# HilaManor/AudioEditingCode

Measured on AMD Instinct MI355X. Metric: edited-clips/sec (200-step inv+edit, 10 s@16 kHz), higher is better.
Workload: dtype f32

## Files before the change

audioeditingcode_amd/csrc/conv_gemm_x6.hip:

```cpp
#include "cg_params.h"

typedef __bf16 bf16x8 __attribute__((ext_vector_type(8)));
typedef __bf16 bf16x2 __attribute__((ext_vector_type(2)));
typedef float f32x2 __attribute__((ext_vector_type(2)));

int launch_conv_gemm_x6(const aed_op* op, hipStream_t s);

constexpr int X6_BK = 16;

__device__ __forceinline__ void x6_split_pair(float x0, float x1, unsigned& h, unsigned& m, unsigned& l) {
    h = __builtin_bit_cast(unsigned, __builtin_convertvector((f32x2){x0, x1}, bf16x2));
    float r0 = x0 - __uint_as_float(h << 16);
    float r1 = x1 - __uint_as_float(h & 0xffff0000u);
    asm volatile("" : "+v"(r0), "+v"(r1));
    m = __builtin_bit_cast(unsigned, __builtin_convertvector((f32x2){r0, r1}, bf16x2));
    float q0 = r0 - __uint_as_float(m << 16);
    float q1 = r1 - __uint_as_float(m & 0xffff0000u);
    asm volatile("" : "+v"(q0), "+v"(q1));
    l = __builtin_bit_cast(unsigned, __builtin_convertvector((f32x2){q0, q1}, bf16x2));
}

typedef unsigned u32x4 __attribute__((ext_vector_type(4)));
constexpr unsigned X6_OOB = 0x80000000u;

template <int G, int NM, int NV>
__device__ __forceinline__ void x6_hints() {
    if constexpr (G < NM) {
        constexpr int v = (NV * (G + 1)) / NM - (NV * G) / NM;
        if constexpr (v > 0) __builtin_amdgcn_sched_group_barrier(0x002, v, 0);
        __builtin_amdgcn_sched_group_barrier(0x008, 1, 0);
        x6_hints<G + 1, NM, NV>();
    }
}

template <int BM, int BN, int WROWS, int WCOLS, int DEPTH, bool PLAIN, int SCHED, int NTERMS, int BK = X6_BK>
__global__ __launch_bounds__(64 * WROWS * WCOLS, 2) void conv_gemm_x6_kernel(CGParams p) {
    constexpr int NT = 64 * WROWS * WCOLS;
    constexpr int WM = BM / WROWS, WN = BN / WCOLS;
    constexpr int TM = WM / 32, TN = WN / 32;
    constexpr int TPR = BK / 4;
    constexpr int RPP = NT / TPR;
    constexpr int PA = BM / RPP, PB = BN / RPP;
    constexpr int PQ = BK / 8;
    constexpr int X6_ROWQ = 3 * PQ + 1;
    constexpr int KB = BK / 16;
    constexpr int STAGE = (BM + BN) * X6_ROWQ;
    static_assert(BK == 16 || BK == 32, "chunk width");
    static_assert(TM >= 1 && TN >= 1 && PA >= 1 && PB >= 1, "tile");
    static_assert(BM % RPP == 0 && BN % RPP == 0, "loader passes");

    __shared__ uint4 lds[2 * STAGE];
    const unsigned nx = gridDim.x, ny = gridDim.y, bz = blockIdx.z, gz = gridDim.z;
    const unsigned orig = blockIdx.y * nx + blockIdx.x;

    const int tid = threadIdx.x;
    const int lane = tid & 63;
    const int wave = tid >> 6;
    const int wr = wave / WCOLS, wc = wave % WCOLS;
    int tile_y = (int)(orig / nx), tile_x = (int)(orig - (unsigned)tile_y * nx);
    if (gz == 1) {
        const unsigned nwg = nx * ny;
        const unsigned xcd = orig & 7u, q = nwg >> 3, r = nwg & 7u;
        const unsigned id = (xcd < r ? xcd * (q + 1) : r * (q + 1) + (xcd - r) * q) + (orig >> 3);
        if (p.gm > 1) {
            const unsigned per_group = (unsigned)p.gm * nx;
            const unsigned g = id / per_group, first = g * (unsigned)p.gm;
            const unsigned gsz = min((unsigned)p.gm, ny - first);
            const unsigned within = id - g * per_group;
            tile_x = (int)(within / gsz);
            tile_y = (int)(first + (within - (unsigned)tile_x * gsz));
        } else {
            tile_y = (int)(id / nx);
            tile_x = (int)(id - (unsigned)tile_y * nx);
        }
    }
    const int m0 = tile_y * BM;
    const int n0 = tile_x * BN;

    int kc_begin = 0, kc_end = p.nchunks;
    if (p.ksplit > 1) {
        const int per = (p.nchunks + p.ksplit - 1) / p.ksplit;
        kc_begin = (int)bz * per;
        kc_end = min(p.nchunks, kc_begin + per);
    }

    const int lrow = tid / TPR;
    const int lq = tid % TPR;
    const int lcol = lq * 4;

    int ay0[PA], ax0[PA];
    unsigned abase[PA], abase2[PA];
    bool avalid[PA];
#pragma unroll
    for (int q = 0; q < PA; ++q) {
        const int m = m0 + lrow + RPP * q;
        avalid[q] = m < p.M;
        const int mm = avalid[q] ? m : 0;
        int b = 0, r = mm, oy = mm, ox = 0;
        if (p.rpb != p.M || p.OW != 1) {
            b = mm / p.rpb;
            r = mm - b * p.rpb;
            oy = r / p.OW;
            ox = r - oy * p.OW;
        }
        ay0[q] = oy * p.stride - p.pad_h;
        ax0[q] = ox * p.stride - p.pad_w;
        abase[q] = (unsigned)b * (unsigned)p.a_bs + lcol;
        abase2[q] = (unsigned)b * (unsigned)p.a_bs2 + lcol;
    }
    unsigned wbase[PB];
    bool wvalid[PB];
#pragma unroll
    for (int q = 0; q < PB; ++q) {
        const int n = n0 + lrow + RPP * q;
        wvalid[q] = n < p.N;
        wbase[q] = (unsigned)(wvalid[q] ? n : 0) * (unsigned)p.K + lcol;
    }
    const int vIH = p.vIH, vIW = p.vIW;
    int pf_cg, pf_sub, pf_ty, pf_tx;
    const int gq = p.kgroup / BK;
    if (kc_begin == 0) {
        pf_cg = pf_sub = pf_ty = pf_tx = 0;
    } else {
        const int per_group = p.KH * p.KW * gq;
        const int g = kc_begin / per_group;
        const int rem = kc_begin - g * per_group;
        const int tap = rem / gq;
        pf_cg = g * p.kgroup;
        pf_sub = rem - tap * gq;
        pf_ty = tap / p.KW;
        pf_tx = tap - pf_ty * p.KW;
    }

    float4 rbuf_a[DEPTH][PA], rbuf_b[DEPTH][PB];
    float ln_s1[PA], ln_s2[PA];
#pragma unroll
    for (int q = 0; q < PA; ++q) { ln_s1[q] = 0.f; ln_s2[q] = 0.f; }

    const __amdgpu_buffer_rsrc_t srd_a = __builtin_amdgcn_make_buffer_rsrc((void*)p.A, 0, 0x7ffffff0, 0x00020000);
    const __amdgpu_buffer_rsrc_t srd_a2 = __builtin_amdgcn_make_buffer_rsrc((void*)(p.A2 ? p.A2 : p.A), 0, 0x7ffffff0, 0x00020000);
    const __amdgpu_buffer_rsrc_t srd_w = __builtin_amdgcn_make_buffer_rsrc((void*)p.W, 0, 0x7ffffff0, 0x00020000);
    auto as_f4 = [](u32x4 v) {
        return make_float4(__uint_as_float(v.x), __uint_as_float(v.y), __uint_as_float(v.z), __uint_as_float(v.w));
    };
    auto prefetch = [&](int kc, float4 (&ra)[PA], float4 (&rb)[PB]) {
        int c0 = pf_cg + pf_sub * BK;
        const int dy = pf_ty * p.dil_h, dx = pf_tx * p.dil_w;
        const unsigned k0 = (unsigned)((pf_ty * p.KW + pf_tx) * p.Cin + c0);
        pf_sub += 1;
        const bool wrap = pf_sub == gq;
        pf_sub = wrap ? 0 : pf_sub;
        pf_tx += wrap ? 1 : 0;
        const bool wrap2 = pf_tx == p.KW;
        pf_tx = wrap2 ? 0 : pf_tx;
        pf_ty += wrap2 ? 1 : 0;
        const bool wrap3 = pf_ty == p.KH;
        pf_ty = wrap3 ? 0 : pf_ty;
        pf_cg += wrap3 ? p.kgroup : 0;
        const bool second = p.C1 > 0 && c0 >= p.C1;
        c0 -= second ? p.C1 : 0;
        const unsigned ld = second ? (unsigned)p.lda2 : (unsigned)p.lda;
        const bool dead = kc >= kc_end;
#pragma unroll
        for (int q = 0; q < PA; ++q) {
            const int iy = ay0[q] + dy, ix = ax0[q] + dx;
            const bool ok = avalid[q] & ((unsigned)iy < (unsigned)vIH) & ((unsigned)ix < (unsigned)vIW) & !dead;
            const unsigned base = second ? abase2[q] : abase[q];
            const unsigned off = (base + (unsigned)((iy >> p.up) * p.IW + (ix >> p.up)) * ld + (unsigned)c0) * 4u;
            ra[q] = as_f4(__builtin_amdgcn_raw_buffer_load_b128(second ? srd_a2 : srd_a, ok ? off : X6_OOB, 0, 0));
        }
#pragma unroll
        for (int q = 0; q < PB; ++q)
            rb[q] = as_f4(__builtin_amdgcn_raw_buffer_load_b128(
                srd_w, (wvalid[q] & !dead) ? (wbase[q] + k0) * 4u : X6_OOB, 0, 0));
    };

    auto put_row = [&](uint4* st, int row, float4 v, bool is_w = false) {
        unsigned h0, m0_, l0, h1, m1, l1;
#ifdef X6_DIAG_NOSPLIT
        if (X6_DIAG_NOSPLIT == 2 || is_w) {
            h0 = __builtin_bit_cast(unsigned, __builtin_convertvector((f32x2){v.x, v.y}, bf16x2));
            h1 = __builtin_bit_cast(unsigned, __builtin_convertvector((f32x2){v.z, v.w}, bf16x2));
            m0_ = l0 = h0;
            m1 = l1 = h1;
        } else
#endif
        {
            x6_split_pair(v.x, v.y, h0, m0_, l0);
            x6_split_pair(v.z, v.w, h1, m1, l1);
        }
        uint2* dst = reinterpret_cast<uint2*>(st + row * X6_ROWQ) + lq;
        dst[0] = make_uint2(h0, h1);
        dst[2 * PQ] = make_uint2(m0_, m1);
        dst[4 * PQ] = make_uint2(l0, l1);
    };

    auto stage_write = [&](uint4* st, const float4 (&ra)[PA], const float4 (&rb)[PB]) {
#pragma unroll
        for (int q = 0; q < PA; ++q) {
            float4 v = ra[q];
            if constexpr (!PLAIN) {
                if (p.ln_mode) {
                    ln_s1[q] += (v.x + v.y) + (v.z + v.w);
                    ln_s2[q] += (v.x * v.x + v.y * v.y) + (v.z * v.z + v.w * v.w);
                }
                if (p.in_act) {
                    v.x = in_transform(v.x, p.in_act, p.in_slope);
                    v.y = in_transform(v.y, p.in_act, p.in_slope);
                    v.z = in_transform(v.z, p.in_act, p.in_slope);
                    v.w = in_transform(v.w, p.in_act, p.in_slope);
                }
            }
            put_row(st, lrow + RPP * q, v);
        }
#pragma unroll
        for (int q = 0; q < PB; ++q) put_row(st, BM + lrow + RPP * q, rb[q], true);
    };

    f32x16 acc[TM][TN];
#pragma unroll
    for (int a = 0; a < TM; ++a)
#pragma unroll
        for (int b = 0; b < TN; ++b)
#pragma unroll
            for (int r = 0; r < 16; ++r) acc[a][b][r] = 0.f;

    const int fi = lane & 31;
    const int fh = lane >> 5;
    const int a_frag = (wr * WM + fi) * X6_ROWQ + fh;
    const int b_frag = (BM + wc * WN + fi) * X6_ROWQ + fh;

    bf16x8 af[TM][3], bw[TN][3];
    auto load_frags = [&](const uint4* st, int kb, bf16x8 (&fa)[TM][3], bf16x8 (&fb)[TN][3]) {
#pragma unroll
        for (int a = 0; a < TM; ++a)
#pragma unroll
            for (int pl = 0; pl < 3; ++pl)
                fa[a][pl] = __builtin_bit_cast(bf16x8, st[a_frag + a * 32 * X6_ROWQ + PQ * pl + 2 * kb]);
#pragma unroll
        for (int b = 0; b < TN; ++b)
#pragma unroll
            for (int pl = 0; pl < 3; ++pl)
                fb[b][pl] = __builtin_bit_cast(bf16x8, st[b_frag + b * 32 * X6_ROWQ + PQ * pl + 2 * kb]);
    };
    auto do_mfmas = [&](const bf16x8 (&fa)[TM][3], const bf16x8 (&fb)[TN][3]) {
        constexpr int TA[6] = {0, 2, 1, 0, 1, 0};
        constexpr int TB[6] = {2, 0, 1, 1, 0, 0};
#pragma unroll
        for (int t = 6 - NTERMS; t < 6; ++t)
#pragma unroll
            for (int a = 0; a < TM; ++a)
#pragma unroll
                for (int b = 0; b < TN; ++b)
                    acc[a][b] = __builtin_amdgcn_mfma_f32_32x32x16_bf16(fa[a][TA[t]], fb[b][TB[t]], acc[a][b], 0, 0, 0);
    };
    auto hints = [&]() {
        if constexpr (SCHED == 1) {
            constexpr int NM = TM * TN * NTERMS * KB;
            x6_hints<0, NM, NM * (((PA + PB) * 22 + 40 + NM - 1) / NM)>();
        }
    };

#pragma unroll
    for (int d = 0; d < DEPTH; ++d) prefetch(kc_begin + d, rbuf_a[d], rbuf_b[d]);
    stage_write(lds, rbuf_a[0], rbuf_b[0]);
    prefetch(kc_begin + DEPTH, rbuf_a[0], rbuf_b[0]);
    __syncthreads();
    int cur = 0;
    for (int kc0 = kc_begin; kc0 < kc_end; kc0 += DEPTH) {
#pragma unroll
        for (int d = 0; d < DEPTH; ++d) {
            const int kc = kc0 + d;
            const int sl = (d + 1) % DEPTH;
            load_frags(lds + cur * STAGE, 0, af, bw);
            stage_write(lds + (cur ^ 1) * STAGE, rbuf_a[sl], rbuf_b[sl]);
            prefetch(kc + 1 + DEPTH, rbuf_a[sl], rbuf_b[sl]);
            do_mfmas(af, bw);
            if constexpr (KB == 2) {
                bf16x8 af2[TM][3], bw2[TN][3];
                load_frags(lds + cur * STAGE, 1, af2, bw2);
                do_mfmas(af2, bw2);
            }
            hints();
            __syncthreads();
            cur ^= 1;
        }
    }

    float* ln_stat = reinterpret_cast<float*>(lds);
#include "cg_epilogue.h"
}

template <int BM, int BN, int WR, int WC, int DEPTH, bool DIAG, int BK = X6_BK>
static int x6_launch(const CGParams& p, bool plain, int sched, int terms, hipStream_t s) {
    dim3 grid(aed_cdiv(p.N, BN), aed_cdiv(p.M, BM), p.ksplit);
    dim3 block(64 * WR * WC);
#define X6_GO(PL, SC, NT_) hipLaunchKernelGGL((conv_gemm_x6_kernel<BM, BN, WR, WC, DEPTH, PL, SC, NT_, BK>), grid, block, 0, s, p)
    if (terms == 3) {
        if constexpr (DIAG) {
            if (plain) { X6_GO(true, 1, 3); return 0; }
        }
        AED_REQUIRE(false, "conv_gemm_x6: the three-term diagnostic exists for tiles 1 and 8 with a plain A operand");
    }
    if (!plain) X6_GO(false, 1, 6);
    else if (sched) X6_GO(true, 1, 6);
    else X6_GO(true, 0, 6);
#undef X6_GO
    return 0;
}

int launch_conv_gemm_x6(const aed_op* op, hipStream_t s) {
    const int32_t* i = op->i;
    const int Cin = i[11];
    int cfg = i[29];
    const long long batch = i[0] / (i[9] * i[10] > 0 ? i[9] * i[10] : 1);
    const bool fits = (Cin % X6_BK == 0) && (i[3] % 4 == 0) && ((uintptr_t)op->p[0] % 16 == 0) &&
                      ((uintptr_t)op->p[1] % 16 == 0) && cfg < 10 && cfg != 5 && cfg != 6 && cfg != 7 && i[36] == 0 &&
                      i[37] == 0 && i[38] <= 1 && i[39] == 0 &&
                      batch * i[20] + (long long)i[7] * i[8] * i[3] < (1LL << 29) && (long long)i[1] * i[2] < (1LL << 29) &&
                      (i[32] == 0 || batch * i[34] + (long long)i[7] * i[8] * i[33] < (1LL << 29));
    if (!fits) {
        if (cfg == 8 || cfg == 9) {
            aed_op fp32_op = *op;
            fp32_op.i[29] = 1;
            return launch_conv_gemm(&fp32_op, s);
        }
        return launch_conv_gemm(op, s);
    }
    const bool wide = (op->flags & 256) && (cfg == 8 || cfg == 9) && Cin % 32 == 0 && !(op->flags & 16);
    CGParams p;
    int rc = cg_fill_params(op, p, wide ? 32 : X6_BK);
    if (rc) return rc;
    if (p.ksplit > (p.K + 31) / 32) p.ksplit = (p.K + 31) / 32;
    if (cfg == 0) {
        const int cus = aed_num_cus();
        auto blocks = [&](int bm, int bn) { return (long)aed_cdiv(p.M, bm) * aed_cdiv(p.N, bn) * p.ksplit; };
        if (p.N >= 512 && p.N % 256 == 0 && blocks(128, 256) >= 2L * cus) cfg = 9;
        else if (blocks(256, 128) >= 2L * cus && p.N >= 128) cfg = 8;
        else if (blocks(128, 128) >= (long)cus && p.N >= 128) cfg = 1;
        else if (blocks(128, 64) >= 2L * cus) cfg = 2;
        else cfg = 4;
    }
    if (!(op->flags & 1024) && p.ksplit <= 1) {
        static const int BMs[10] = {0, 128, 128, 64, 64, 0, 0, 0, 256, 128}, BNs[10] = {0, 128, 64, 128, 64, 0, 0, 0, 128, 256};
        const int nx = aed_cdiv(p.N, BNs[cfg]), ny = aed_cdiv(p.M, BMs[cfg]);
        const int resident = ((aed_num_cus() >> ((op->flags >> 16) & 3)) / 8) * ((cfg == 8 || cfg == 9) ? 1 : 2);
        if (nx > 1 && ny > 1) {
            int g = 1;
            while (g * 2 <= ny && (long)(g * 2) * (g * 2) * BMs[cfg] <= (long)resident * BNs[cfg]) g *= 2;
            if (resident / g < nx) p.gm = g;
            if (op->flags & 0x3800) p.gm = 1 << ((op->flags >> 11) & 7);
        }
    }
    const bool plain = p.in_act == 0 && p.ln_mode == 0;
    const int sched = (op->flags & 8) ? 1 : 0;
    const int terms = (op->flags & 16) ? 3 : 6;
    if (p.geglu) AED_REQUIRE(cfg == 1 || cfg == 3 || cfg == 8 || cfg == 9, "conv_gemm_x6: the GEGLU epilogue needs 64-wide wave tiles (cfg %d)", cfg);
    switch (cfg) {
        case 1: rc = x6_launch<128, 128, 2, 2, 2, true>(p, plain, sched, terms, s); break;
        case 2: rc = x6_launch<128, 64, 2, 2, 2, false>(p, plain, sched, terms, s); break;
        case 3: rc = x6_launch<64, 128, 2, 2, 2, false>(p, plain, sched, terms, s); break;
        case 4: rc = x6_launch<64, 64, 2, 2, 2, false>(p, plain, sched, terms, s); break;
        case 8: rc = wide && terms == 6 ? x6_launch<256, 128, 4, 2, 2, false, 32>(p, plain, sched, terms, s)
                                        : x6_launch<256, 128, 4, 2, 2, true>(p, plain, sched, terms, s); break;
        case 9: rc = wide && terms == 6 ? x6_launch<128, 256, 2, 4, 2, false, 32>(p, plain, sched, terms, s)
                                        : x6_launch<128, 256, 2, 4, 2, false>(p, plain, sched, terms, s); break;
        default: AED_REQUIRE(false, "conv_gemm_x6: bad tile cfg %d", cfg);
    }
    if (rc) return rc;
    AED_CHECK_HIP(hipGetLastError());
    if (p.ksplit > 1) return launch_splitk_reduce(op, s);
    return 0;
}
```

audioeditingcode_amd/tile_table_x6_cus64.py:

```python
TILE_TABLE = {
    (2, 512, 128, 0): (10, 1),
    (2, 512, 512, 0): (12, 1),
    (2, 8320, 512, 0): (10, 1),
    (128, 384, 3456, 0): (104, 16),
    (128, 640, 384, 0): (10, 1),
    (128, 640, 640, 0): (10, 1),
    (128, 640, 1024, 0): (104, 8),
    (128, 640, 1280, 0): (104, 8),
    (128, 640, 3200, 0): (104, 8),
    (128, 640, 3456, 0): (103, 16),
    (128, 640, 5760, 0): (103, 16),
    (128, 640, 9216, 0): (103, 16),
    (128, 640, 11520, 0): (103, 16),
    (128, 1920, 640, 0): (15, 1),
    (128, 5120, 640, 1): (103, 1),
    (512, 256, 2304, 0): (103, 8),
    (512, 384, 256, 0): (10, 1),
    (512, 384, 384, 0): (10, 1),
    (512, 384, 640, 0): (10, 1),
    (512, 384, 768, 0): (10, 1),
    (512, 384, 1024, 0): (104, 4),
    (512, 384, 1920, 0): (103, 8),
    (512, 384, 2304, 0): (103, 8),
    (512, 384, 3456, 0): (103, 8),
    (512, 384, 5760, 0): (103, 8),
    (512, 384, 6912, 0): (103, 8),
    (512, 384, 9216, 0): (103, 8),
    (512, 640, 5760, 0): (103, 8),
    (512, 1152, 384, 0): (104, 1),
    (512, 3072, 384, 1): (103, 1),
    (2048, 128, 1152, 0): (103, 4),
    (2048, 256, 128, 0): (104, 1),
    (2048, 256, 256, 0): (104, 1),
    (2048, 256, 384, 0): (104, 1),
    (2048, 256, 512, 0): (104, 1),
    (2048, 256, 640, 0): (104, 1),
    (2048, 256, 1152, 0): (103, 2),
    (2048, 256, 1280, 0): (103, 2),
    (2048, 256, 2304, 0): (103, 4),
    (2048, 256, 3456, 0): (103, 4),
    (2048, 256, 4608, 0): (103, 8),
    (2048, 256, 5760, 0): (103, 8),
    (2048, 384, 3456, 0): (103, 2),
    (2048, 768, 256, 0): (103, 1),
    (2048, 2048, 256, 1): (109, 1),
    (8192, 8, 1152, 0): (10, 1),
    (8192, 128, 72, 0): (4, 1),
    (8192, 128, 256, 0): (103, 1),
    (8192, 128, 384, 0): (103, 1),
    (8192, 128, 1152, 0): (103, 1),
    (8192, 128, 2304, 0): (103, 1),
    (8192, 128, 3456, 0): (103, 1),
    (8192, 256, 2304, 0): (109, 1),
}
```

audioeditingcode_amd/tile_table_x6_cus64_b1.py:

```python
TILE_TABLE = {
    (1, 512, 128, 0): (10, 1),
    (1, 512, 512, 0): (10, 1),
    (1, 8320, 512, 0): (10, 1),
    (64, 384, 3456, 0): (104, 16),
    (64, 640, 384, 0): (12, 1),
    (64, 640, 640, 0): (12, 1),
    (64, 640, 1024, 0): (11, 1),
    (64, 640, 1280, 0): (11, 1),
    (64, 640, 3200, 0): (104, 16),
    (64, 640, 3456, 0): (104, 16),
    (64, 640, 5760, 0): (103, 32),
    (64, 640, 9216, 0): (103, 32),
    (64, 640, 11520, 0): (104, 16),
    (64, 1920, 640, 0): (10, 1),
    (64, 5120, 640, 1): (13, 1),
    (256, 256, 2304, 0): (104, 8),
    (256, 384, 256, 0): (10, 1),
    (256, 384, 384, 0): (10, 1),
    (256, 384, 640, 0): (10, 1),
    (256, 384, 768, 0): (10, 1),
    (256, 384, 1024, 0): (104, 8),
    (256, 384, 1920, 0): (104, 8),
    (256, 384, 2304, 0): (104, 8),
    (256, 384, 3456, 0): (103, 16),
    (256, 384, 5760, 0): (103, 16),
    (256, 384, 6912, 0): (103, 16),
    (256, 384, 9216, 0): (103, 16),
    (256, 640, 5760, 0): (103, 16),
    (256, 1152, 384, 0): (104, 1),
    (256, 3072, 384, 1): (103, 1),
    (1024, 128, 1152, 0): (104, 4),
    (1024, 256, 128, 0): (104, 1),
    (1024, 256, 256, 0): (104, 1),
    (1024, 256, 384, 0): (104, 1),
    (1024, 256, 512, 0): (104, 1),
    (1024, 256, 640, 0): (15, 1),
    (1024, 256, 1152, 0): (103, 4),
    (1024, 256, 1280, 0): (103, 4),
    (1024, 256, 2304, 0): (103, 4),
    (1024, 256, 3456, 0): (103, 4),
    (1024, 256, 4608, 0): (103, 8),
    (1024, 256, 5760, 0): (103, 8),
    (1024, 384, 3456, 0): (103, 4),
    (1024, 768, 256, 0): (104, 1),
    (1024, 2048, 256, 1): (109, 1),
    (4096, 8, 1152, 0): (10, 1),
    (4096, 128, 72, 0): (4, 1),
    (4096, 128, 256, 0): (104, 1),
    (4096, 128, 384, 0): (104, 1),
    (4096, 128, 1152, 0): (104, 1),
    (4096, 128, 2304, 0): (104, 1),
    (4096, 128, 3456, 0): (104, 1),
    (4096, 256, 2304, 0): (103, 1),
}
```

Measured before the change: 0.9764.

## Add intra-block K-split wave groups to small x6 conv GEMM tiles

Adds a WK template parameter so that, for small-grid 64-row tiles (cfg 3/4, no ksplit, at most 64 blocks), a block runs two wave groups that each take half of the K chunks in separate LDS stages. At the end, the second group writes its accumulators and LayerNorm partial sums to LDS and group 0 adds them before the epilogue. The goal is more parallelism on under-filled GPUs without a second kernel or atomics, at the cost of larger blocks, extra LDS traffic and a reduction barrier. Several tile-table entries are retuned to pick the configurations that now use this path.

Measured after the change: 0.9810, median of 3. About the same (+0.5%).

```diff
diff --git a/audioeditingcode_amd/csrc/conv_gemm_x6.hip b/audioeditingcode_amd/csrc/conv_gemm_x6.hip
--- a/audioeditingcode_amd/csrc/conv_gemm_x6.hip
+++ b/audioeditingcode_amd/csrc/conv_gemm_x6.hip
@@ -33,8 +33,8 @@
     }
 }
 
-template <int BM, int BN, int WROWS, int WCOLS, int DEPTH, bool PLAIN, int SCHED, int NTERMS, int BK = X6_BK>
-__global__ __launch_bounds__(64 * WROWS * WCOLS, 2) void conv_gemm_x6_kernel(CGParams p) {
+template <int BM, int BN, int WROWS, int WCOLS, int DEPTH, bool PLAIN, int SCHED, int NTERMS, int BK = X6_BK, int WK = 1>
+__global__ __launch_bounds__(64 * WROWS * WCOLS * WK, 2) void conv_gemm_x6_kernel(CGParams p) {
     constexpr int NT = 64 * WROWS * WCOLS;
     constexpr int WM = BM / WROWS, WN = BN / WCOLS;
     constexpr int TM = WM / 32, TN = WN / 32;
@@ -48,12 +48,17 @@
     static_assert(BK == 16 || BK == 32, "chunk width");
     static_assert(TM >= 1 && TN >= 1 && PA >= 1 && PB >= 1, "tile");
     static_assert(BM % RPP == 0 && BN % RPP == 0, "loader passes");
-
-    __shared__ uint4 lds[2 * STAGE];
+    static_assert(WK == 1 || WK == 2, "K groups");
+    constexpr int KG_PER_THREAD = TM * TN * 16 + 2 * PA;
+    static_assert(WK == 1 || (2 * BM + (WK - 1) * NT * KG_PER_THREAD) * 4 <= WK * 2 * STAGE * 16, "K-group hand-over fits the stages");
+
+    __shared__ uint4 lds_all[WK * 2 * STAGE];
+    const int grp = WK > 1 ? __builtin_amdgcn_readfirstlane((int)threadIdx.x / NT) : 0;
+    uint4* const lds = lds_all + grp * (2 * STAGE);
     const unsigned nx = gridDim.x, ny = gridDim.y, bz = blockIdx.z, gz = gridDim.z;
     const unsigned orig = blockIdx.y * nx + blockIdx.x;
 
-    const int tid = threadIdx.x;
+    const int tid = WK > 1 ? (int)threadIdx.x - grp * NT : (int)threadIdx.x;
     const int lane = tid & 63;
     const int wave = tid >> 6;
     const int wr = wave / WCOLS, wc = wave % WCOLS;
@@ -83,6 +88,13 @@
         kc_begin = (int)bz * per;
         kc_end = min(p.nchunks, kc_begin + per);
     }
+    int kc_loop_end = kc_end;
+    if constexpr (WK > 1) {
+        const int per = (max(kc_end - kc_begin, 0) + WK - 1) / WK;
+        kc_begin += grp * per;
+        kc_loop_end = kc_begin + per;
+        kc_end = min(kc_end, kc_loop_end);
+    }
 
     const int lrow = tid / TPR;
     const int lq = tid % TPR;
@@ -267,7 +279,7 @@
     prefetch(kc_begin + DEPTH, rbuf_a[0], rbuf_b[0]);
     __syncthreads();
     int cur = 0;
-    for (int kc0 = kc_begin; kc0 < kc_end; kc0 += DEPTH) {
+    for (int kc0 = kc_begin; kc0 < kc_loop_end; kc0 += DEPTH) {
 #pragma unroll
         for (int d = 0; d < DEPTH; ++d) {
             const int kc = kc0 + d;
@@ -287,26 +299,78 @@
         }
     }
 
+    if constexpr (WK > 1) {
+        float* const kg = reinterpret_cast<float*>(lds_all) + 2 * BM;
+        if (grp > 0) {
+            float* dst = kg + (grp - 1) * (NT * KG_PER_THREAD) + tid;
+#pragma unroll
+            for (int a = 0; a < TM; ++a)
+#pragma unroll
+                for (int b = 0; b < TN; ++b)
+#pragma unroll
+                    for (int r = 0; r < 16; ++r) dst[((a * TN + b) * 16 + r) * NT] = acc[a][b][r];
+            if constexpr (!PLAIN) {
+#pragma unroll
+                for (int q = 0; q < PA; ++q) {
+                    dst[(TM * TN * 16 + 2 * q) * NT] = ln_s1[q];
+                    dst[(TM * TN * 16 + 2 * q + 1) * NT] = ln_s2[q];
+                }
+            }
+        }
+        __syncthreads();
+        if (grp > 0) {
+            if (p.ln_mode) __syncthreads();
+            return;
+        }
+#pragma unroll
+        for (int g = 1; g < WK; ++g) {
+            const float* src = kg + (g - 1) * (NT * KG_PER_THREAD) + tid;
+#pragma unroll
+            for (int a = 0; a < TM; ++a)
+#pragma unroll
+                for (int b = 0; b < TN; ++b)
+#pragma unroll
+                    for (int r = 0; r < 16; ++r) acc[a][b][r] += src[((a * TN + b) * 16 + r) * NT];
+            if constexpr (!PLAIN) {
+#pragma unroll
+                for (int q = 0; q < PA; ++q) {
+                    ln_s1[q] += src[(TM * TN * 16 + 2 * q) * NT];
+                    ln_s2[q] += src[(TM * TN * 16 + 2 * q + 1) * NT];
+                }
+            }
+        }
+    }
     float* ln_stat = reinterpret_cast<float*>(lds);
 #include "cg_epilogue.h"
 }
 
-template <int BM, int BN, int WR, int WC, int DEPTH, bool DIAG, int BK = X6_BK>
+template <int BM, int BN, int WR, int WC, int DEPTH, bool DIAG, int BK = X6_BK, int WK = 1>
 static int x6_launch(const CGParams& p, bool plain, int sched, int terms, hipStream_t s) {
     dim3 grid(aed_cdiv(p.N, BN), aed_cdiv(p.M, BM), p.ksplit);
-    dim3 block(64 * WR * WC);
-#define X6_GO(PL, SC, NT_) hipLaunchKernelGGL((conv_gemm_x6_kernel<BM, BN, WR, WC, DEPTH, PL, SC, NT_, BK>), grid, block, 0, s, p)
-    if (terms == 3) {
-        if constexpr (DIAG) {
-            if (plain) { X6_GO(true, 1, 3); return 0; }
-        }
-        AED_REQUIRE(false, "conv_gemm_x6: the three-term diagnostic exists for tiles 1 and 8 with a plain A operand");
-    }
-    if (!plain) X6_GO(false, 1, 6);
-    else if (sched) X6_GO(true, 1, 6);
-    else X6_GO(true, 0, 6);
+    dim3 block(64 * WR * WC * WK);
+#define X6_GO(PL, SC, NT_) hipLaunchKernelGGL((conv_gemm_x6_kernel<BM, BN, WR, WC, DEPTH, PL, SC, NT_, BK, WK>), grid, block, 0, s, p)
+    if constexpr (WK > 1) {
+        AED_REQUIRE(terms == 6 && sched, "conv_gemm_x6: the K-group forms need flag bit 3 and six terms");
+        if (plain) X6_GO(true, 1, 6);
+        else X6_GO(false, 1, 6);
+    } else {
+        if (terms == 3) {
+            if constexpr (DIAG) {
+                if (plain) { X6_GO(true, 1, 3); return 0; }
+            }
+            AED_REQUIRE(false, "conv_gemm_x6: the three-term diagnostic exists for tiles 1 and 8 with a plain A operand");
+        }
+        if (!plain) X6_GO(false, 1, 6);
+        else if (sched) X6_GO(true, 1, 6);
+        else X6_GO(true, 0, 6);
+    }
 #undef X6_GO
     return 0;
+}
+
+static bool x6_kgroup_rule(int cfg, int M, int N, int ksplit) {
+    if ((cfg != 3 && cfg != 4) || ksplit > 1 || M > 512) return false;
+    return (long)aed_cdiv(M, 64) * aed_cdiv(N, cfg == 3 ? 128 : 64) <= 64;
 }
 
 int launch_conv_gemm_x6(const aed_op* op, hipStream_t s) {
@@ -355,12 +419,16 @@
     const bool plain = p.in_act == 0 && p.ln_mode == 0;
     const int sched = (op->flags & 8) ? 1 : 0;
     const int terms = (op->flags & 16) ? 3 : 6;
-    if (p.geglu) AED_REQUIRE(cfg == 1 || cfg == 3 || cfg == 8 || cfg == 9, "conv_gemm_x6: the GEGLU epilogue needs 64-wide wave tiles (cfg %d)", cfg);
+    const bool kgroups = x6_kgroup_rule(cfg, p.M, p.N, p.ksplit) && sched && terms == 6 && !(op->flags & 0x40000);
+    if (p.geglu) AED_REQUIRE(cfg == 1 || cfg == 3 || cfg == 8 || cfg == 9 || (cfg == 4 && kgroups),
+                             "conv_gemm_x6: the GEGLU epilogue needs 64-wide wave tiles (cfg %d)", cfg);
     switch (cfg) {
         case 1: rc = x6_launch<128, 128, 2, 2, 2, true>(p, plain, sched, terms, s); break;
         case 2: rc = x6_launch<128, 64, 2, 2, 2, false>(p, plain, sched, terms, s); break;
-        case 3: rc = x6_launch<64, 128, 2, 2, 2, false>(p, plain, sched, terms, s); break;
-        case 4: rc = x6_launch<64, 64, 2, 2, 2, false>(p, plain, sched, terms, s); break;
+        case 3: rc = kgroups ? x6_launch<64, 128, 2, 2, 2, false, X6_BK, 2>(p, plain, sched, terms, s)
+                             : x6_launch<64, 128, 2, 2, 2, false>(p, plain, sched, terms, s); break;
+        case 4: rc = kgroups ? x6_launch<64, 64, 2, 1, 2, false, X6_BK, 2>(p, plain, sched, terms, s)
+                             : x6_launch<64, 64, 2, 2, 2, false>(p, plain, sched, terms, s); break;
         case 8: rc = wide && terms == 6 ? x6_launch<256, 128, 4, 2, 2, false, 32>(p, plain, sched, terms, s)
                                         : x6_launch<256, 128, 4, 2, 2, true>(p, plain, sched, terms, s); break;
         case 9: rc = wide && terms == 6 ? x6_launch<128, 256, 2, 4, 2, false, 32>(p, plain, sched, terms, s)
diff --git a/audioeditingcode_amd/tile_table_x6_cus64.py b/audioeditingcode_amd/tile_table_x6_cus64.py
--- a/audioeditingcode_amd/tile_table_x6_cus64.py
+++ b/audioeditingcode_amd/tile_table_x6_cus64.py
@@ -12,7 +12,7 @@
     (128, 640, 5760, 0): (103, 16),
     (128, 640, 9216, 0): (103, 16),
     (128, 640, 11520, 0): (103, 16),
-    (128, 1920, 640, 0): (15, 1),
+    (128, 1920, 640, 0): (104, 1),
     (128, 5120, 640, 1): (103, 1),
     (512, 256, 2304, 0): (103, 8),
     (512, 384, 256, 0): (10, 1),
diff --git a/audioeditingcode_amd/tile_table_x6_cus64_b1.py b/audioeditingcode_amd/tile_table_x6_cus64_b1.py
--- a/audioeditingcode_amd/tile_table_x6_cus64_b1.py
+++ b/audioeditingcode_amd/tile_table_x6_cus64_b1.py
@@ -13,7 +13,7 @@
     (64, 640, 9216, 0): (103, 32),
     (64, 640, 11520, 0): (104, 16),
     (64, 1920, 640, 0): (10, 1),
-    (64, 5120, 640, 1): (13, 1),
+    (64, 5120, 640, 1): (103, 1),
     (256, 256, 2304, 0): (104, 8),
     (256, 384, 256, 0): (10, 1),
     (256, 384, 384, 0): (10, 1),
@@ -27,7 +27,7 @@
     (256, 384, 6912, 0): (103, 16),
     (256, 384, 9216, 0): (103, 16),
     (256, 640, 5760, 0): (103, 16),
-    (256, 1152, 384, 0): (104, 1),
+    (256, 1152, 384, 0): (103, 1),
     (256, 3072, 384, 1): (103, 1),
     (1024, 128, 1152, 0): (104, 4),
     (1024, 256, 128, 0): (104, 1),
```
